# CVMI-Lab/HybridNeuralRendering

Measured on AMD Instinct MI355X. Metric: rays/sec (fwd render) scene0241_01 at 1/2/4/8 GPU; PSNR delta vs ref, higher is better.
Workload: dtype f32

## Files before the change

### hybridneuralrendering_amd/csrc/aggregate.hip

```cpp
#include "hnr_common.h"
#include "hnr_launch.h"

namespace hnr {

__device__ __forceinline__ int count_neighbours(const int32_t *__restrict__ p, int K)
{
    int n = 0;
    while (n < K && p[n] >= 0) ++n;
    return n;
}

__global__ __launch_bounds__(1024) void plan_block_sum_kernel(const int32_t *__restrict__ work, const int32_t *__restrict__ pidx,
                                                              const unsigned long long *__restrict__ counts, int K,
                                                              int32_t *__restrict__ block_sums)
{
    __shared__ int s_a[16], s_b[16];
    const int n_items = (int)counts[HNR_CNT_SAMPLES];
    const int i = blockIdx.x * 1024 + threadIdx.x;
    int nb = i < n_items ? count_neighbours(pidx + (size_t)work[i] * K, K) : 0;
    int v = nb > 0;
    for (int o = 32; o > 0; o >>= 1) { nb += __shfl_xor(nb, o); v += __shfl_xor(v, o); }
    if ((threadIdx.x & 63) == 0) { s_a[threadIdx.x >> 6] = v; s_b[threadIdx.x >> 6] = nb; }
    __syncthreads();
    if (threadIdx.x == 0) {
// ... 485 lines not shown
            wv *= vm[u];
            if (a.frame_w) wv *= a.frame_w[v0 + u];
            fsum += f[u] * wv;
            wsum += wv;
        }
    }
    float *o = a.X7 + (size_t)s * a.ld7;
    if (lane < 45) {
        o[lane] = a.CF[(size_t)s * a.ldcf + lane];
        const bool drop = a.ray_drop && a.ray_drop[a.vs_item[s] / a.SR];
        o[45 + lane] = drop ? 0.f : hnr_div(fsum, wsum + 1e-6f);
    }
    }
}

struct FinalArgs {
    const float *Y; int ldy;
    const float *CF; int ldcf;
    const float *w_fin, *b_fin;
    const float *sigma;
    const int32_t *vs_item;
    const unsigned long long *counts;
    float *decoded;
};

__global__ __launch_bounds__(256) void final_color_kernel(FinalArgs a)
{
    const int lane = threadIdx.x & 63, l16 = lane & 15, sub = lane >> 4;
    const int n_valid = (int)a.counts[HNR_CNT_SAMPLES_VALID];
    float w[3][8];
#pragma unroll
    for (int j = 0; j < 3; ++j)
#pragma unroll
        for (int e = 0; e < 8; ++e) w[j][e] = a.w_fin[j * 128 + 8 * l16 + e];
    const float b0 = a.b_fin[0], b1 = a.b_fin[1], b2 = a.b_fin[2];
    const bool yvec = a.ldy >= 48 && (a.ldy & 3) == 0 && (reinterpret_cast<uintptr_t>(a.Y) & 15) == 0;
    const int wave_g = (int)((blockIdx.x * (unsigned)blockDim.x + threadIdx.x) >> 6), n_waves = (int)((gridDim.x * (unsigned)blockDim.x) >> 6);
    for (int s0 = 4 * wave_g; s0 < n_valid; s0 += 4 * n_waves) {
        const int s = s0 + sub;
        const bool ok = s < n_valid;
        const size_t sc = ok ? (size_t)s : (size_t)(n_valid - 1);
        const float4 c0 = *reinterpret_cast<const float4 *>(a.CF + sc * a.ldcf + 8 * l16), c1 = *reinterpret_cast<const float4 *>(a.CF + sc * a.ldcf + 8 * l16 + 4);
        float x[8] = {c0.x, c0.y, c0.z, c0.w, c1.x, c1.y, c1.z, c1.w};
        if (yvec) {
            if (l16 < 6) {
                const float4 y0 = *reinterpret_cast<const float4 *>(a.Y + sc * a.ldy + 8 * l16), y1 = *reinterpret_cast<const float4 *>(a.Y + sc * a.ldy + 8 * l16 + 4);
                const float y[8] = {y0.x, y0.y, y0.z, y0.w, y1.x, y1.y, y1.z, y1.w};
#pragma unroll
                for (int e = 0; e < 8; ++e) if (8 * l16 + e < 45) x[e] = y[e] + x[e];
            }
        } else {
#pragma unroll
            for (int e = 0; e < 8; ++e) {
                const int c = 8 * l16 + e;
                if (c < 45) x[e] = a.Y[sc * a.ldy + c] + x[e];
            }
        }
        float r[3] = {0.f, 0.f, 0.f};
#pragma unroll
        for (int j = 0; j < 3; ++j) {
#pragma unroll
            for (int e = 0; e < 8; ++e) r[j] += x[e] * w[j][e];
            r[j] += __builtin_amdgcn_update_dpp(0.f, r[j], 0xB1, 0xf, 0xf, false);
            r[j] += __builtin_amdgcn_update_dpp(0.f, r[j], 0x4E, 0xf, 0xf, false);
            r[j] += __builtin_amdgcn_update_dpp(0.f, r[j], 0x141, 0xf, 0xf, false);
            r[j] += __builtin_amdgcn_update_dpp(0.f, r[j], 0x140, 0xf, 0xf, false);
        }
        if (l16 == 0 && ok) {
            float4 out;
            out.x = a.sigma[s];
            const float bb[3] = {b0, b1, b2};
            float rgb[3];
#pragma unroll
            for (int j = 0; j < 3; ++j) {
                const float sg = hnr_div(1.f, 1.f + expf(-(r[j] + bb[j])));
                rgb[j] = sg * (1.f + 2.f * 0.001f) - 0.001f;
            }
            out.y = rgb[0]; out.z = rgb[1]; out.w = rgb[2];
            reinterpret_cast<float4 *>(a.decoded)[a.vs_item[s]] = out;
        }
    }
}

struct CompositeArgs {
    const float *decoded;
    const float *loc_w;
    const int32_t *pidx;
    const int8_t *ray_mask;
    const int32_t *nsamp;
    const float *campos, *camrot, *bg;
    int R, SR, K;
    float vsize_z;
    int unit_mode;
    float *raycolor;
    float *opacity;
    float *is_bg;
    float *blend_w;
};

__global__ __launch_bounds__(256) void composite_kernel(CompositeArgs a)
{
    const int r = blockIdx.x * blockDim.x + threadIdx.x;
    if (r >= a.R) return;
    const float bg0 = a.bg[0], bg1 = a.bg[1], bg2 = a.bg[2];
    float *op = a.opacity + (size_t)r * a.SR;
    if (!a.ray_mask[r]) {
        a.raycolor[3 * (size_t)r] = bg0; a.raycolor[3 * (size_t)r + 1] = bg1; a.raycolor[3 * (size_t)r + 2] = bg2;
        a.is_bg[r] = 1.f;
        for (int s = 0; s < a.SR; ++s) { op[s] = 0.f; if (a.blend_w) a.blend_w[(size_t)r * a.SR + s] = 0.f; }
        return;
    }
    float cr[9];
#pragma unroll
    for (int i = 0; i < 9; ++i) cr[i] = a.camrot[i];
    const float cp[3] = {a.campos[0], a.campos[1], a.campos[2]};
    const int ns = a.nsamp ? a.nsamp[r] : a.SR;
    auto zc = [&](int s) {
        const float *p = a.loc_w + ((size_t)r * a.SR + s) * 3;
        const float q0 = s < ns ? p[0] : 0.f, q1 = s < ns ? p[1] : 0.f, q2 = s < ns ? p[2] : 0.f;
        const float s0 = __fsub_rn(q0, cp[0]), s1 = __fsub_rn(q1, cp[1]), s2 = __fsub_rn(q2, cp[2]);
        return __fadd_rn(__fadd_rn(__fmul_rn(cr[2], s0), __fmul_rn(cr[5], s1)), __fmul_rn(cr[8], s2));
    };
    float T = 1.f, c0 = 0.f, c1 = 0.f, c2 = 0.f;
    float zmax = zc(0);
    const int s_end = ns < a.SR ? ns : a.SR;
    for (int s = s_end; s < a.SR; ++s) { op[s] = 0.f; if (a.blend_w) a.blend_w[(size_t)r * a.SR + s] = 0.f; }
    for (int s = 0; s < s_end; ++s) {
        float dist;
        if (s + 1 < a.SR) {
            const float zn = fmaxf(zmax, zc(s + 1));
            dist = __fsub_rn(zn, zmax);
            zmax = zn;
        } else {
            dist = a.vsize_z;
        }
        if (dist < 1e-8f || (a.unit_mode && dist > 2.f * a.vsize_z)) dist = a.vsize_z;
        const bool valid = s < ns && a.pidx[((size_t)r * a.SR + s) * a.K] >= 0;
        const float4 d = reinterpret_cast<const float4 *>(a.decoded)[(size_t)r * a.SR + s];
        const float sigma = valid ? d.x : 0.f;
        const float rd = valid ? dist : 0.f;
        const float o = 1.f - expf(-sigma * rd);
        const float bw = o * T;
        c0 += d.y * bw; c1 += d.z * bw; c2 += d.w * bw;
        op[s] = o;
        if (a.blend_w) a.blend_w[(size_t)r * a.SR + s] = bw;
        T *= (1.f - o + 1e-10f);
    }
    a.raycolor[3 * (size_t)r] = c0 + bg0 * T;
    a.raycolor[3 * (size_t)r + 1] = c1 + bg1 * T;
    a.raycolor[3 * (size_t)r + 2] = c2 + bg2 * T;
    a.is_bg[r] = T;
}

__global__ __launch_bounds__(256) void ray_march_kernel(const float *__restrict__ ray_dist, const uint8_t *__restrict__ ray_valid,
                                                        const float *__restrict__ feat , const float *__restrict__ bg ,
                                                        int R, int SR, float *__restrict__ ray_color, float *__restrict__ opacity,
                                                        float *__restrict__ acc_t, float *__restrict__ blend_w, float *__restrict__ bg_t)
{
    const int r = blockIdx.x * blockDim.x + threadIdx.x;
    if (r >= R) return;
    float T = 1.f, c0 = 0.f, c1 = 0.f, c2 = 0.f;
    for (int s = 0; s < SR; ++s) {
        const size_t i = (size_t)r * SR + s;
        const float4 d = reinterpret_cast<const float4 *>(feat)[i];
        const float sigma = ray_valid[i] ? d.x : 0.f;
        const float o = 1.f - expf(-sigma * ray_dist[i]);
        const float w = o * T;
        opacity[i] = o; acc_t[i] = T; blend_w[i] = w;
        c0 += d.y * w; c1 += d.z * w; c2 += d.w * w;
        T *= (1.f - o + 1e-10f);
    }
    if (bg) { c0 += bg[0] * T; c1 += bg[1] * T; c2 += bg[2] * T; }
    ray_color[3 * (size_t)r] = c0; ray_color[3 * (size_t)r + 1] = c1; ray_color[3 * (size_t)r + 2] = c2;
    bg_t[r] = T;
}

struct ProbeArgs {
    const float *opacity, *loc_w;
    const int32_t *pidx;
    const float *weight, *conf_c;
    const float *xyz, *emb, *conf, *pdir, *color;
    int F, R, SR, K;
    float *o_opacity, *o_loc, *o_far, *o_color, *o_dir, *o_conf, *o_emb;
};

__global__ __launch_bounds__(256) void probe_kernel(ProbeArgs a)
{
    const int64_t t = (int64_t)blockIdx.x * blockDim.x + threadIdx.x;
    const int r = (int)(t >> 3), sub = (int)(t & 7);
    if (r >= a.R) return;
    int best = 0;
    float bo = a.opacity[(size_t)r * a.SR];
    for (int s = 1; s < a.SR; ++s) {
        const float o = a.opacity[(size_t)r * a.SR + s];
        if (o > bo) { bo = o; best = s; }
    }
    const size_t item = (size_t)r * a.SR + best;
    const float lx = a.loc_w[3 * item], ly = a.loc_w[3 * item + 1], lz = a.loc_w[3 * item + 2];
    float far = INFINITY, acc_c[3] = {0.f, 0.f, 0.f}, acc_d[3] = {0.f, 0.f, 0.f}, acc_f = 0.f;
    float acc_e[4] = {0.f, 0.f, 0.f, 0.f};
    for (int k = 0; k < a.K; ++k) {
        const int raw = a.pidx[item * a.K + k];
        const int pid = raw < 0 ? 0 : raw;
        const float w = a.weight[item * a.K + k] * a.conf_c[item * a.K + k];
        const float dx = a.xyz[3 * (size_t)pid] - lx, dy = a.xyz[3 * (size_t)pid + 1] - ly, dz = a.xyz[3 * (size_t)pid + 2] - lz;
        far = fminf(far, sqrtf(dx * dx + dy * dy + dz * dz));
#pragma unroll
        for (int j = 0; j < 3; ++j) {
            acc_c[j] += a.color[3 * (size_t)pid + j] * w;
            acc_d[j] += a.pdir[3 * (size_t)pid + j] * w;
        }
        acc_f += a.conf[pid] * w;
#pragma unroll
        for (int q = 0; q < 4; ++q) {
            const int c = sub + 8 * q;
            if (c < a.F) acc_e[q] += a.emb[(size_t)pid * a.F + c] * w;
        }
    }
#pragma unroll
    for (int q = 0; q < 4; ++q) {
        const int c = sub + 8 * q;
        if (c < a.F) a.o_emb[(size_t)r * a.F + c] = acc_e[q];
    }
    if (sub == 0) {
        a.o_opacity[r] = bo; a.o_far[r] = far; a.o_conf[r] = acc_f;
        a.o_loc[3 * (size_t)r] = lx; a.o_loc[3 * (size_t)r + 1] = ly; a.o_loc[3 * (size_t)r + 2] = lz;
#pragma unroll
        for (int j = 0; j < 3; ++j) { a.o_color[3 * (size_t)r + j] = acc_c[j]; a.o_dir[3 * (size_t)r + j] = acc_d[j]; }
    }
}

__global__ __launch_bounds__(256) void gather_points_kernel(const int32_t *__restrict__ pidx, int64_t n, const float *__restrict__ xyz,
                                                            const float *__restrict__ emb, const float *__restrict__ conf,
                                                            const float *__restrict__ pdir, const float *__restrict__ color, int F,
                                                            const float *__restrict__ campos, const float *__restrict__ camrot,
                                                            float *__restrict__ o_color, float *__restrict__ o_dir,
                                                            float *__restrict__ o_conf, float *__restrict__ o_emb,
                                                            float *__restrict__ o_pers, float *__restrict__ o_xyz, uint8_t *__restrict__ o_mask)
{
    const int64_t e = ((int64_t)blockIdx.x * blockDim.x + threadIdx.x) >> 3;
    const int sub = threadIdx.x & 7;
    if (e >= n) return;
    const int raw = pidx[e];
    const int pid = raw < 0 ? 0 : raw;
    for (int c = sub; c < F; c += 8) o_emb[e * F + c] = emb[(size_t)pid * F + c];
    if (sub < 3) {
        o_color[e * 3 + sub] = color[3 * (size_t)pid + sub];
        o_dir[e * 3 + sub] = pdir[3 * (size_t)pid + sub];
        o_xyz[e * 3 + sub] = xyz[3 * (size_t)pid + sub];
    }
    if (sub == 3) {
        const float p[3] = {xyz[3 * (size_t)pid], xyz[3 * (size_t)pid + 1], xyz[3 * (size_t)pid + 2]};
        float pp[3];
        w2pers(p, campos, camrot, pp);
        o_pers[e * 3] = pp[0]; o_pers[e * 3 + 1] = pp[1]; o_pers[e * 3 + 2] = pp[2];
    }
    if (sub == 4) { o_conf[e] = conf[pid]; o_mask[e] = raw >= 0 ? 1 : 0; }
}

}

using namespace hnr;

extern "C" int hnr_gather_points(const int32_t *d_sample_pidx, int64_t n_entries, const float *d_xyz, const float *d_emb,
                                 const float *d_conf, const float *d_dir, const float *d_color, int F, const float *d_campos,
                                 const float *d_camrot, float *d_o_color, float *d_o_dir, float *d_o_conf, float *d_o_emb,
                                 float *d_o_xyz_pers, float *d_o_xyz, uint8_t *d_o_mask, void *stream)
{
    if (n_entries < 0 || F <= 0) { set_error("hnr_gather_points: bad sizes"); return HNR_ERR_BADARG; }
    if (n_entries == 0) return HNR_OK;
    if (!d_sample_pidx || !d_xyz || !d_emb || !d_conf || !d_dir || !d_color || !d_campos || !d_camrot || !d_o_color || !d_o_dir ||
        !d_o_conf || !d_o_emb || !d_o_xyz_pers || !d_o_xyz || !d_o_mask) {
        set_error("hnr_gather_points: NULL argument"); return HNR_ERR_BADARG;
    }
    gather_points_kernel<<<cdiv(n_entries * 8, 256), 256, 0, (hipStream_t)stream>>>(d_sample_pidx, n_entries, d_xyz, d_emb, d_conf, d_dir,
                                                                                   d_color, F, d_campos, d_camrot, d_o_color, d_o_dir,
                                                                                   d_o_conf, d_o_emb, d_o_xyz_pers, d_o_xyz, d_o_mask);
    HNR_LAUNCH_CHECK();
    return HNR_OK;
}

extern "C" int hnr_sample_plan(const int32_t *d_work, const int32_t *d_sample_pidx, const int64_t *d_counts, int K,
                               int max_items, int32_t *d_vs_item, int32_t *d_vs_off, int32_t *d_vs_cnt,
                               int cap_samples, int cap_rows, int32_t *d_scratch, int32_t *d_overflow, void *stream)
{
    if (!d_work || !d_sample_pidx || !d_counts || !d_vs_item || !d_vs_off || !d_vs_cnt || !d_scratch || !d_overflow ||
        K <= 0 || max_items < 0) {
        set_error("hnr_sample_plan: bad argument"); return HNR_ERR_BADARG;
    }
    hipStream_t st = (hipStream_t)stream;
    HNR_HIP_CHECK(hipMemsetAsync(d_overflow, 0, 4, st));
    if (max_items == 0) return HNR_OK;
    const int nb = cdiv(max_items, 1024);
    const unsigned long long *cnt = reinterpret_cast<const unsigned long long *>(d_counts);
    plan_block_sum_kernel<<<nb, 1024, 0, st>>>(d_work, d_sample_pidx, cnt, K, d_scratch);
    plan_scan_kernel<<<nb, 1024, 0, st>>>(d_work, d_sample_pidx, cnt, K, d_scratch, d_vs_item, d_vs_off, d_vs_cnt,
                                          cap_samples, cap_rows, d_overflow);
    HNR_LAUNCH_CHECK();
    return HNR_OK;
}

extern "C" int hnr_gather_rows(const float *d_xyz, const float *d_emb, const float *d_conf, const float *d_dir,
                               const float *d_color, int F, const int32_t *d_sample_pidx, const float *d_sample_loc_w,
                               const float *d_raydir, const float *d_campos, const float *d_camrot,
                               const int32_t *d_vs_item, const int32_t *d_vs_off, const int32_t *d_vs_cnt,
                               const int64_t *d_counts, int SR, int K, int cap_samples,
// ... 146 lines not shown
    float *s2a = s1 + (size_t)V * 6 * H1 * W1, *s2 = s2a + (size_t)V * 12 * H2 * W2;
    float *s3a = s2 + (size_t)V * 12 * H2 * W2, *s3 = s3a + (size_t)V * 24 * H3 * W3;
    static const int old_conv = knob("HNR_CONV_OLD", 0);
    auto conv = [&](const float *in, int Cin, int Hin, int Win, int cl, int cstride, int li, int Cout, int stride, int Hout, int Wout, float *out) {
        const int64_t total = (int64_t)V * Cout * Hout * Wout, pixels = (int64_t)V * Hout * Wout;
#define HNR_CONV_TILE(CIN_, CT_, CL_) \
        if (!old_conv && Cin == CIN_ && Cout % CT_ == 0 && cl == CL_) { \
            conv3x3_lrelu_tile_kernel<CIN_, CT_, CL_><<<dim3((unsigned)cdiv(pixels, 256), Cout / CT_), 256, 0, st>>>(in, Hin, Win, cstride, d_conv_w[li], d_conv_b[li], \
                                                                                                                 Cout, stride, Hout, Wout, slope, out, V); \
            return; }
        HNR_CONV_TILE(3, 6, 1) HNR_CONV_TILE(6, 6, 0) HNR_CONV_TILE(12, 6, 0) HNR_CONV_TILE(24, 6, 0)
#undef HNR_CONV_TILE
        conv3x3_lrelu_kernel<<<cdiv(total, 256), 256, 0, st>>>(in, Cin, Hin, Win, cl, cstride, d_conv_w[li], d_conv_b[li], Cout, stride,
                                                                Hout, Wout, slope, out, V);
    };
    conv(d_img, 3, H, W, 1, 3, 0, 6, 2, H1, W1, s1a);
    conv(s1a, 6, H1, W1, 0, 0, 1, 6, 1, H1, W1, s1);
    conv(s1, 6, H1, W1, 0, 0, 2, 12, 2, H2, W2, s2a);
    conv(s2a, 12, H2, W2, 0, 0, 3, 12, 1, H2, W2, s2);
    conv(s2, 12, H2, W2, 0, 0, 4, 24, 2, H3, W3, s3a);
    conv(s3a, 24, H3, W3, 0, 0, 5, 24, 1, H3, W3, s3);
    featmap_kernel<<<dim3((unsigned)cdiv((int64_t)V * H * W, 256), 4), 256, 0, st>>>(d_img, s1, s2, s3, V, H, W, H1, W1, H2, W2, H3, W3, d_featmap);
    HNR_LAUNCH_CHECK();
    return HNR_OK;
}

extern "C" int64_t hnr_image_features_scratch_elems(int V, int H, int W)
{
    auto o = [](int n) { return (n + 2 - 3) / 2 + 1; };
    const int64_t H1 = o(H), W1 = o(W), H2 = o((int)H1), W2 = o((int)W1), H3 = o((int)H2), W3 = o((int)W2);
    return 2 * (int64_t)V * (6 * H1 * W1 + 12 * H2 * W2 + 24 * H3 * W3);
}

extern "C" int hnr_proj_rows(const float *d_sample_loc_w, const int32_t *d_vs_item, const int64_t *d_counts, const float *d_w2c,
                             const float *d_intrinsic, const float *d_campos, const float *d_campos_nearest, const float *d_featmap,
                             int V, int H, int W, const float *d_CF, int ldcf, int cap_samples, float *d_X6, int ld6,
                             float *d_vmask, int32_t *d_row_sample, void *stream)
{
    const bool split = d_row_sample != nullptr;
    if (!d_sample_loc_w || !d_vs_item || !d_counts || !d_w2c || !d_intrinsic || !d_campos || !d_campos_nearest || !d_featmap ||
        (!split && !d_CF) || !d_X6 || !d_vmask || V <= 0 || ld6 < (split ? 48 : 176) || (ld6 & 3) || (!split && (ldcf < 128 || (ldcf & 3)))) {
        set_error("hnr_proj_rows: bad argument"); return HNR_ERR_BADARG;
    }
    if (cap_samples <= 0) return HNR_OK;
    ProjArgs a;
    a.loc_w = d_sample_loc_w; a.vs_item = d_vs_item; a.counts = reinterpret_cast<const unsigned long long *>(d_counts);
    a.w2c = d_w2c; a.Kmat = d_intrinsic; a.campos = d_campos; a.campos_n = d_campos_nearest; a.fm = d_featmap; a.H = H; a.W = W;
    a.CF = d_CF; a.ldcf = ldcf; a.V = V; a.cap = cap_samples; a.X6 = d_X6; a.ld6 = ld6; a.vmask = d_vmask; a.row_sample = d_row_sample;
    { const int need = cdiv((int64_t)V * cap_samples * 16, 256); proj_rows_kernel<<<need < 8192 ? need : 8192, 256, 0, (hipStream_t)stream>>>(a); }
    HNR_LAUNCH_CHECK();
    return HNR_OK;
}

__global__ void div_probe_kernel(const float *n, const float *d, int count, float *q_hnr, float *q_ieee)
{
    const int i = blockIdx.x * blockDim.x + threadIdx.x;
    if (i < count) { q_hnr[i] = hnr::hnr_div(n[i], d[i]); q_ieee[i] = n[i] / d[i]; }
}
extern "C" int hnr_div_probe(const float *d_num, const float *d_den, int n, float *d_q_hnr, float *d_q_ieee, void *stream)
{
    if (n < 0 || (n > 0 && (!d_num || !d_den || !d_q_hnr || !d_q_ieee))) { set_error("hnr_div_probe: bad argument"); return HNR_ERR_BADARG; }
    if (n == 0) return HNR_OK;
    div_probe_kernel<<<cdiv(n, 256), 256, 0, (hipStream_t)stream>>>(d_num, d_den, n, d_q_hnr, d_q_ieee);
    HNR_LAUNCH_CHECK();
    return HNR_OK;
}

__global__ void div_probe2_kernel(const float *__restrict__ p, const float *__restrict__ c, float o, int count, int32_t *__restrict__ cell_hnr, int32_t *__restrict__ cell_ieee,
                                  double *__restrict__ q64_hnr, double *__restrict__ q64_ieee)
{
    const int i = blockIdx.x * blockDim.x + threadIdx.x;
    if (i >= count) return;
    cell_hnr[i] = hnr::cell_coord(p[i], o, c[i]);
    const float q = __fsub_rn(p[i], o) / c[i];
    cell_ieee[i] = (q > -2.0e9f && q < 2.0e9f) ? (int)floorf(q) : INT32_MIN;
    const double n = (double)p[i] * 1.0000001192092896, d = (double)c[i] * 3.0000000000000004;
    q64_hnr[i] = hnr::hnr_div64(n, d); q64_ieee[i] = n / d;
}
extern "C" int hnr_div_probe2(const float *d_p, const float *d_c, float origin, int n, int32_t *d_cell_hnr, int32_t *d_cell_ieee, double *d_q64_hnr, double *d_q64_ieee,
                              void *stream)
{
    if (n < 0 || (n > 0 && (!d_p || !d_c || !d_cell_hnr || !d_cell_ieee || !d_q64_hnr || !d_q64_ieee))) { set_error("hnr_div_probe2: bad argument"); return HNR_ERR_BADARG; }
    if (n == 0) return HNR_OK;
    div_probe2_kernel<<<cdiv(n, 256), 256, 0, (hipStream_t)stream>>>(d_p, d_c, origin, n, d_cell_hnr, d_cell_ieee, d_q64_hnr, d_q64_ieee);
    HNR_LAUNCH_CHECK();
    return HNR_OK;
}

extern "C" int hnr_proj_pixels(const float *d_sample_loc_w, const int32_t *d_vs_item, const int64_t *d_counts, const float *d_w2c,
                               const float *d_intrinsic, int V, int H, int W, int cap_samples, int32_t *d_pix, void *stream)
{
    if (!d_sample_loc_w || !d_vs_item || !d_counts || !d_w2c || !d_intrinsic || !d_pix || V <= 0 || H <= 0 || W <= 0) {
        set_error("hnr_proj_pixels: bad argument"); return HNR_ERR_BADARG;
    }
    if (cap_samples <= 0) return HNR_OK;
    const int need = cdiv((int64_t)V * cap_samples, 256);
    proj_pixels_kernel<<<need < 8192 ? need : 8192, 256, 0, (hipStream_t)stream>>>(d_sample_loc_w, d_vs_item, reinterpret_cast<const unsigned long long *>(d_counts), d_w2c,
                                                                                      d_intrinsic, V, H, W, cap_samples, d_pix);
    HNR_LAUNCH_CHECK();
    return HNR_OK;
}

extern "C" int hnr_merge(const float *d_X6, int ld6, const float *d_Hm, int ldh, const float *d_w_last, const float *d_b_last,
                         const float *d_vmask, const float *d_frame_w, const float *d_CF, int ldcf, const int64_t *d_counts,
                         int V, int cap_samples, float *d_X7, int ld7, const uint8_t *d_ray_drop, const int32_t *d_vs_item, int SR,
                         void *stream)
{
    if (!d_X6 || !d_Hm || !d_w_last || !d_b_last || !d_vmask || !d_CF || !d_counts || !d_X7 || ldh < 64 || ld7 < 90 ||
        (d_ray_drop && (!d_vs_item || SR <= 0))) {
        set_error("hnr_merge: bad argument"); return HNR_ERR_BADARG;
    }
    if (cap_samples <= 0) return HNR_OK;
    MergeArgs a;
    a.X6 = d_X6; a.ld6 = ld6; a.Hm = d_Hm; a.ldh = ldh; a.w_last = d_w_last; a.b_last = d_b_last; a.vmask = d_vmask;
    a.frame_w = d_frame_w; a.CF = d_CF; a.ldcf = ldcf; a.counts = reinterpret_cast<const unsigned long long *>(d_counts);
    a.V = V; a.cap = cap_samples; a.X7 = d_X7; a.ld7 = ld7; a.ray_drop = d_ray_drop; a.vs_item = d_vs_item; a.SR = SR;
    { const int need = cdiv((int64_t)cap_samples * 64, 256); merge_kernel<<<need < 8192 ? need : 8192, 256, 0, (hipStream_t)stream>>>(a); }
    HNR_LAUNCH_CHECK();
    return HNR_OK;
}

extern "C" int hnr_final_color(const float *d_Y, int ldy, const float *d_CF, int ldcf, const float *d_w_fin, const float *d_b_fin,
                               const float *d_sigma, const int32_t *d_vs_item, const int64_t *d_counts, int cap_samples,
                               float *d_decoded, void *stream)
{
    if (!d_Y || !d_CF || !d_w_fin || !d_b_fin || !d_sigma || !d_vs_item || !d_counts || !d_decoded || ldy < 45 || ldcf < 128 || (ldcf & 3) ||
        ((uintptr_t)d_CF & 15)) {
        set_error("hnr_final_color: bad argument (NULL pointer, ldy < 45, ldcf < 128 or not a multiple of 4, colour feature not 16-B aligned)"); return HNR_ERR_BADARG;
    }
    if (cap_samples <= 0) return HNR_OK;
    FinalArgs a;
    a.Y = d_Y; a.ldy = ldy; a.CF = d_CF; a.ldcf = ldcf; a.w_fin = d_w_fin; a.b_fin = d_b_fin; a.sigma = d_sigma;
    a.vs_item = d_vs_item; a.counts = reinterpret_cast<const unsigned long long *>(d_counts); a.decoded = d_decoded;
    { const int need = cdiv((int64_t)cap_samples * 16, 256); final_color_kernel<<<need < 8192 ? need : 8192, 256, 0, (hipStream_t)stream>>>(a); }
    HNR_LAUNCH_CHECK();
    return HNR_OK;
}

extern "C" int hnr_composite(const float *d_decoded, const float *d_sample_loc_w, const int32_t *d_sample_pidx,
                             const int8_t *d_ray_mask, const int32_t *d_ray_nsamp, const float *d_campos, const float *d_camrot, const float *d_bg_color,
                             int R, int SR, int K, float vsize_z, int raydist_mode_unit, float *d_raycolor, float *d_opacity,
                             float *d_is_background, float *d_blend_weight, void *stream)
{
    if (R < 0 || SR <= 0 || K <= 0) { set_error("hnr_composite: bad sizes"); return HNR_ERR_BADARG; }
    if (R == 0) return HNR_OK;
    if (!d_decoded || !d_sample_loc_w || !d_sample_pidx || !d_ray_mask || !d_campos || !d_camrot || !d_bg_color || !d_raycolor ||
        !d_opacity || !d_is_background) {
        set_error("hnr_composite: NULL argument"); return HNR_ERR_BADARG;
    }
    CompositeArgs a;
    a.decoded = d_decoded; a.loc_w = d_sample_loc_w; a.pidx = d_sample_pidx; a.ray_mask = d_ray_mask; a.nsamp = d_ray_nsamp; a.campos = d_campos;
    a.camrot = d_camrot; a.bg = d_bg_color; a.R = R; a.SR = SR; a.K = K; a.vsize_z = vsize_z; a.unit_mode = raydist_mode_unit;
    a.raycolor = d_raycolor; a.opacity = d_opacity; a.is_bg = d_is_background; a.blend_w = d_blend_weight;
    composite_kernel<<<cdiv(R, 256), 256, 0, (hipStream_t)stream>>>(a);
    HNR_LAUNCH_CHECK();
    return HNR_OK;
}

extern "C" int hnr_ray_march(const float *d_ray_dist, const uint8_t *d_ray_valid, const float *d_features, const float *d_bg_color, int R,
                             int SR, float *d_ray_color, float *d_opacity, float *d_acc_transmission, float *d_blend_weight,
                             float *d_bg_transmission, void *stream)
{
    if (R < 0 || SR <= 0) { set_error("hnr_ray_march: bad sizes"); return HNR_ERR_BADARG; }
    if (R == 0) return HNR_OK;
    if (!d_ray_dist || !d_ray_valid || !d_features || !d_ray_color || !d_opacity || !d_acc_transmission || !d_blend_weight || !d_bg_transmission) {
        set_error("hnr_ray_march: NULL argument"); return HNR_ERR_BADARG;
    }
    ray_march_kernel<<<cdiv(R, 256), 256, 0, (hipStream_t)stream>>>(d_ray_dist, d_ray_valid, d_features, d_bg_color, R, SR, d_ray_color, d_opacity,
                                                                    d_acc_transmission, d_blend_weight, d_bg_transmission);
    HNR_LAUNCH_CHECK();
    return HNR_OK;
}

extern "C" int hnr_probe_outputs(const float *d_opacity, const float *d_sample_loc_w, const int32_t *d_sample_pidx, const float *d_weight,
                                 const float *d_conf_coefficient, const float *d_xyz, const float *d_emb, const float *d_conf, const float *d_dir,
                                 const float *d_color, int F, int R, int SR, int K, float *d_max_opacity, float *d_max_loc_w, float *d_far_dist,
                                 float *d_avg_color, float *d_avg_dir, float *d_avg_conf, float *d_avg_emb, void *stream)
{
    if (R < 0 || SR <= 0 || K <= 0 || F <= 0 || F > 32) { set_error("hnr_probe_outputs: bad sizes (F <= 32)"); return HNR_ERR_BADARG; }
    if (R == 0) return HNR_OK;
    if (!d_opacity || !d_sample_loc_w || !d_sample_pidx || !d_weight || !d_conf_coefficient || !d_xyz || !d_emb || !d_conf || !d_dir || !d_color ||
        !d_max_opacity || !d_max_loc_w || !d_far_dist || !d_avg_color || !d_avg_dir || !d_avg_conf || !d_avg_emb) {
        set_error("hnr_probe_outputs: NULL argument"); return HNR_ERR_BADARG;
    }
    ProbeArgs a;
    a.opacity = d_opacity; a.loc_w = d_sample_loc_w; a.pidx = d_sample_pidx; a.weight = d_weight; a.conf_c = d_conf_coefficient; a.xyz = d_xyz;
    a.emb = d_emb; a.conf = d_conf; a.pdir = d_dir; a.color = d_color; a.F = F; a.R = R; a.SR = SR; a.K = K; a.o_opacity = d_max_opacity;
    a.o_loc = d_max_loc_w; a.o_far = d_far_dist; a.o_color = d_avg_color; a.o_dir = d_avg_dir; a.o_conf = d_avg_conf; a.o_emb = d_avg_emb;
    probe_kernel<<<cdiv((int64_t)R * 8, 256), 256, 0, (hipStream_t)stream>>>(a);
    HNR_LAUNCH_CHECK();
    return HNR_OK;
}

namespace hnr {
int point_rows_dc(const float *d_emb, const int32_t *d_ids, int n_cap, const long long *d_n, float *d_E, int lde, hipStream_t st)
{
    if (n_cap <= 0) return HNR_OK;
    const int64_t total = (int64_t)n_cap * (32 / 4 + 3 * 32);
    int blocks = cdiv(total, 256);
    if (blocks > 256 * 16) blocks = 256 * 16;
    point_rows_kernel<32><<<blocks, 256, 0, st>>>(d_emb, d_ids, n_cap, d_E, lde, d_n);
    HNR_LAUNCH_CHECK();
    return HNR_OK;
}
}
```

### hybridneuralrendering_amd/csrc/chain_ws.hip

```cpp
#include <utility>

#include "chain_defs.h"
#include "hnr_launch.h"

namespace hnr {

constexpr int CW_CST = ch_lds_exch(4) + 2048;
constexpr int CW_CST_FLOATS = CH_META_DESCALE + 4;
constexpr int CW_DSUM = CW_CST + ((CW_CST_FLOATS * 4 + 15) & ~15);
constexpr int CW_HMAX = CW_DSUM + 4 * 32 * 4 * 4;
constexpr int cw_lds_bytes() { return CW_HMAX + 5 * 512; }

#define CW_LOAD_FRAG(N_, rsrc_, voff_, soff_, IMM_) asm volatile("buffer_load_dwordx4 a[%2:%3], %0, %1, %4 offen offset:%5" :: "v"(voff_), "s"(rsrc_), "n"(N_), "n"((N_) + 3), "s"(soff_), "n"(IMM_))
template <int N> __device__ __forceinline__ void cw_mfma(f32x16 &acc, const u32x4 &x)
{
    asm volatile("v_mfma_f32_32x32x16_f16 %0, a[%2:%3], %1, %0" : "+v"(acc) : "v"(x), "n"(N), "n"(N + 3));
}
template <int N> __device__ __forceinline__ void cw_mfma_first(f32x16 &acc, const u32x4 &x)
{
    asm volatile("v_mfma_f32_32x32x16_f16 %0, a[%2:%3], %1, 0" : "=&v"(acc) : "v"(x), "n"(N), "n"(N + 3));
}
__device__ __forceinline__ void cw_mfma_vw(f32x16 &acc, const u32x4 &w, const u32x4 &x)
{
    asm volatile("v_mfma_f32_32x32x16_f16 %0, %1, %2, %0" : "+v"(acc) : "v"(w), "v"(x));
// ... 466 lines not shown
            if (ms == 0) {
                if (PR == 3) ex4 = CW_AT_F4(q_dsr, 0);
                const int ls = (j >> (3 - kc_e)) + (4 << kc_e) * PR;
                const bool st = (j & ((8 >> kc_e) - 1)) == 0;
                x5_voff = st ? (ls * a.ld5 + col0) * 4 : 0x40000000;
                x5_flag = kc_e > 0 ? 0.f : 1.f;
                x5_flag2 = kc_e > 1 ? 0.f : 1.f;
                if constexpr (TR) x5m = 0.f;
                if constexpr (TR) x5_take = (st && to.first + CW_KEEP(ls) < to.end) ? 1.f : 0.f;
            } else if (ms < 33) {
                const int d = (ms - 1) >> 2, t = (ms - 1) & 3, c = d >> 2, e0i = 4 * (d & 3), kb = d & 1;
                if (t == 0)
                    asm volatile("v_mul_f32 %0, %4, %8\n\tv_mul_f32 %1, %5, %8\n\tv_mul_f32 %2, %6, %8\n\tv_mul_f32 %3, %7, %8"
                                 : "=&v"(kf[kb][0]), "=&v"(kf[kb][1]), "=&v"(kf[kb][2]), "=&v"(kf[kb][3])
                                 : "v"(acc[se][c][e0i]), "v"(acc[se][c][e0i + 1]), "v"(acc[se][c][e0i + 2]), "v"(acc[se][c][e0i + 3]), "v"(wq_e));
                else if (t == 1)
                    asm volatile("v_add_f32_dpp %0, %0, %0 quad_perm:[1,0,3,2] row_mask:0xf bank_mask:0xf\n\tv_add_f32_dpp %1, %1, %1 quad_perm:[1,0,3,2] row_mask:0xf bank_mask:0xf\n\t"
                                 "v_add_f32_dpp %2, %2, %2 quad_perm:[1,0,3,2] row_mask:0xf bank_mask:0xf\n\tv_add_f32_dpp %3, %3, %3 quad_perm:[1,0,3,2] row_mask:0xf bank_mask:0xf"
                                 : "+v"(kf[kb][0]), "+v"(kf[kb][1]), "+v"(kf[kb][2]), "+v"(kf[kb][3]));
                else if (t == 2)
                    asm volatile("v_fmac_f32_dpp %0, %0, %4 quad_perm:[2,3,0,1] row_mask:0xf bank_mask:0xf\n\tv_fmac_f32_dpp %1, %1, %4 quad_perm:[2,3,0,1] row_mask:0xf bank_mask:0xf\n\t"
                                 "v_fmac_f32_dpp %2, %2, %4 quad_perm:[2,3,0,1] row_mask:0xf bank_mask:0xf\n\tv_fmac_f32_dpp %3, %3, %4 quad_perm:[2,3,0,1] row_mask:0xf bank_mask:0xf"
                                 : "+v"(kf[kb][0]), "+v"(kf[kb][1]), "+v"(kf[kb][2]), "+v"(kf[kb][3]) : "v"(x5_flag2));
                else {
                    asm volatile("v_fmac_f32_dpp %0, %0, %4 row_half_mirror row_mask:0xf bank_mask:0xf\n\tv_fmac_f32_dpp %1, %1, %4 row_half_mirror row_mask:0xf bank_mask:0xf\n\t"
                                 "v_fmac_f32_dpp %2, %2, %4 row_half_mirror row_mask:0xf bank_mask:0xf\n\tv_fmac_f32_dpp %3, %3, %4 row_half_mirror row_mask:0xf bank_mask:0xf"
                                 : "+v"(kf[kb][0]), "+v"(kf[kb][1]), "+v"(kf[kb][2]), "+v"(kf[kb][3]) : "v"(x5_flag));
                    __builtin_amdgcn_raw_buffer_store_b128(u32x4{__float_as_uint(kf[kb][0]), __float_as_uint(kf[kb][1]), __float_as_uint(kf[kb][2]), __float_as_uint(kf[kb][3])}, to.rs,
                                                           x5_voff + (32 * c + e0i) * 4, 0, 0);
                    if constexpr (TR) {
                        const float m4 = fmaxf(fmaxf(fabsf(kf[kb][0]), fabsf(kf[kb][1])), fmaxf(fabsf(kf[kb][2]), fabsf(kf[kb][3])));
                        x5m = fmaxf(x5m, __fmul_rn(m4, x5_take));
                    }
                }
            } else if (ms == 33) {
                if constexpr (TR) CW_HMAX_PUT(4, x5m);
                if (PR == 3) {
                    const float d = __fadd_rn(__fadd_rn(ex4.x, ex4.y), __fadd_rn(ex4.z, ex4.w));
                    __builtin_amdgcn_raw_buffer_store_b32(__float_as_uint(d), to.rs_aux, h == 0 ? (wave * 32 + j) * 4 : 0x40000000, 0, 0);
                }
            } else prefetch_next();
        }
    };

    auto b_read = [&](int rt, int s, int p) __attribute__((always_inline)) {
        const int off = s * SLOT + (rt * 2 + p) * 1024;
        return off < 65536 ? CW_AT(const u32x4, q_b0, off) : off < 131072 ? CW_AT(const u32x4, q_b1, off - 65536) : CW_AT(const u32x4, q_b2, off - 131072);
    };

    TileOut to_fin = tile_out(-1);
    CW_REFRESH(0);
    bq[0] = read_cst(3, 0); bq[1] = read_cst(3, 1); aq[0] = read_cst(4, 0); aq[1] = read_cst(4, 1);
    bf[0][0] = b_read(0, 0, 0); bf[0][1] = b_read(0, 0, 1);
    for (int tile = t_first; tile < t_end; tile += t_step) {
        ++n_my;
        const int tile_next = tile + t_step;
        const int tile_nx = tile_next < t_end ? tile_next : tile;
        const TileOut to_cur = tile_out(tile);
        CW_REFRESH(0);
        bf[1][0] = b_read(0, 1, 0); bf[1][1] = b_read(0, 1, 1);
        cw_static_for<16>([&](auto Pc) __attribute__((always_inline)) {
            constexpr int P = decltype(Pc)::value;
            constexpr int L = P >> 2, rt = P & 3, S = cw_steps(L), G0 = cw_goff(P);
            constexpr int PP = (P + 15) & 15, PL = PP >> 2, PR = PP & 3, sm = rt & 1;
            constexpr int T = 6 * S, H = T / 2;
            const TileOut &to_e = P == 0 ? to_fin : to_cur;
            if (DB >= 2) { const long long t_ = clock64(); tm[(P + 15) & 15] += t_ - t_prev; t_prev = t_; if (P == 2) tmf[3] += t_ - tf_prev; if (P == 1) tf_prev = t_; }
            if constexpr (P != 0) CW_REFRESH(P);
            if (P == 6) {
#pragma unroll
                for (int c = 0; c < 2; ++c)
#pragma unroll
                    for (int p = 0; p < 2; ++p)
                        wx[c][p] = __builtin_bit_cast(u32x4, __builtin_amdgcn_raw_buffer_load_b128(wsrd, woff + (c * 2 + p) * 1024, CH_W2 + 16 * CH_WSTEP, 0));
            }
            if (P == 13) load_ids(tile_nx, pid_n);
            if (P == 1) load_rest(tile);
            __builtin_amdgcn_sched_barrier(0);
            cw_static_for<6 * S>([&](auto kc) __attribute__((always_inline)) {
                constexpr int slot = decltype(kc)::value, it = slot / 6, s = cw_korder(L, it), g = (slot % 6) >> 1, c = slot & 1;
                if (slot == H) {
                    if constexpr (P == 15) { constexpr int d_ = cw_dma_count(0, 15, TR); if constexpr (d_ <= 63) cw_wait_vm<d_>(); }
                    if constexpr (P == 2) { constexpr int d_ = cw_dma_count(3, 2, TR); if constexpr (d_ <= 63) cw_wait_vm<d_>(); }
                    if (DB >= 2 && P == 1) { const long long t_ = clock64(); tmf[0] += t_ - tf_prev; tf_prev = t_; }
                    cw_lds_barrier();
                    if (DB >= 2 && P == 1) { const long long t_ = clock64(); tmf[1] += t_ - tf_prev; tf_prev = t_; }
                    if constexpr (L == 3) dma_image(tile_nx, rt);
                    if constexpr (!TR && L == 0 && rt < 3) load_table(pid[rt + 1], tv[TR ? 0 : (rt + 1) & 1]);
                    if constexpr (TR && L == 0 && rt >= 1) load_table(pid[rt], tv[0]);
                    if constexpr (P == 14) load_table(pid_n[0], tv[0]);
                    if (DB >= 2 && P == 1) { const long long t_ = clock64(); tmf[2] += t_ - tf_prev; tf_prev = t_; }
                    __builtin_amdgcn_sched_barrier(0);
                }
                constexpr int wp = g == 0 ? 1 : 0, xp_ = g == 1 ? 1 : 0;
                constexpr int ring = (G0 + it) % 3;
                if constexpr (rt == 0 && g == 0 && c == 0 && s < 16) {
                    constexpr int n_ = cw_need_count(32 * L + s, P, slot, TR) + (P == 0 ? 8 : 0);
                    if constexpr (n_ <= (TR ? 63 : 56)) cw_wait_vm<n_>();
                }
                constexpr int A0 = 16 * (s < 16 ? s : 0) + 4 * wp + 8 * c;
                if constexpr (DB == 4) { if (slot < 2) { acc[sm][c] = f32x16{} + bf[ring][xp_][0]; } }
                else if constexpr (L == 2 && s == 16) cw_mfma_vw(acc[sm][c], wx[c][wp], bf[ring][xp_]);
                else if constexpr (slot < 2) cw_mfma_first<A0>(acc[sm][c], bf[ring][xp_]);
                else cw_mfma<A0>(acc[sm][c], bf[ring][xp_]);
                __builtin_amdgcn_sched_barrier(0);
                if constexpr (g < 2 && c == 0 && G0 + it + 2 < CW_GTOT) {
                    constexpr int i2 = it + 2 >= S ? it + 2 - S : it + 2, P2 = it + 2 >= S ? P + 1 : P;
                    if constexpr (P2 < 16 && i2 < cw_steps((P2 & 15) >> 2)) bf[(G0 + it + 2) % 3][g] = b_read(P2 & 3, cw_korder((P2 & 15) >> 2, i2), g);
                }
                if constexpr (g < 2 && c == 0 && P == 15 && it == 15) bf[0][g] = b_read(0, 0, g);
                { constexpr int blk = cw_issue(P, slot); if constexpr (blk >= 0) CW_LOAD_W(blk >> 5, blk & 31); }
                if (DB != 3) epilogue_piece(PL, PR, S, slot, to_e);
                __builtin_amdgcn_sched_barrier(0);
            });
        });
        wq_fin = wq[3]; to_fin = to_cur;
#pragma unroll
        for (int rt = 0; rt < 4; ++rt) pid[rt] = pid_n[rt];
    }
    CW_REFRESH(0);
    cw_static_for<6 * CH_S0>([&](auto kc) __attribute__((always_inline)) {
        constexpr int slot = decltype(kc)::value;
        if (slot == (6 * CH_S0) / 2) cw_lds_barrier();
        epilogue_piece(3, 3, CH_S0, slot, to_fin);
    });
    asm volatile("s_waitcnt vmcnt(0)" ::: "memory");
    if constexpr (TR) {
        __syncthreads();
        float *exch = reinterpret_cast<float *>(lds + ch_lds_exch(4));
#pragma unroll
        for (int l = 0; l < 5; ++l) {
            float m = tid < 128 ? CW_LDS(float, CW_HMAX + l * 512 + 4 * tid) : 0.f;
            for (int o = 32; o > 0; o >>= 1) m = fmaxf(m, __shfl_xor(m, o));
            if (lane == 0) exch[4 * l + wave] = m;
        }
        __syncthreads();
        if (tid < 5) {
            const float m = fmaxf(fmaxf(exch[4 * tid], exch[4 * tid + 1]), fmaxf(exch[4 * tid + 2], exch[4 * tid + 3]));
            unsigned *dst = tid < 4 ? (a.hmax ? a.hmax + tid : nullptr) : a.x5max;
            if (dst && m > 0.f) atomicMax(dst, __float_as_uint(m));
        }
    }
    if (DB >= 2 && blockIdx.x == 0 && lane == 0 && a.dbg) {
        long long *o = reinterpret_cast<long long *>(a.dbg) + 4 * 1024 + wave * 16;
        for (int i = 0; i < 16; ++i) o[i] = tm[i];
        if (wave == 0) { long long *o2 = reinterpret_cast<long long *>(a.dbg) + 4 * 1024 + 64; for (int i = 0; i < 4; ++i) o2[i] = tmf[i]; }
    }
    if (DB >= 2 && tid == 0 && a.dbg) {
        long long *o = reinterpret_cast<long long *>(a.dbg) + 4 * (size_t)blockIdx.x;
        o[0] = clock64() - t_start; o[1] = wall_clock64() - w_start; o[2] = n_my; o[3] = 0;
    }
}

__global__ __launch_bounds__(128) void chain_sigma_kernel(ChainArgs a)
{
    const ChainClasses cls = chain_classes(a.counts, a.cap_samples);
    const int tile = blockIdx.x;
    if (tile >= cls.n_tiles) return;
    const int lane = threadIdx.x & 63, rt = threadIdx.x >> 5, j = lane & 31;
    const char *aux = a.aux + ((size_t)tile * 4 + rt) * CH_AUX_GROUP;
    const float d = a.dsig[(size_t)tile * 128 + threadIdx.x], wq = reinterpret_cast<const float *>(aux + 128)[j];
    const float alpha_b = reinterpret_cast<const float *>(a.wimg + CH_META)[4 * 256 + 256];
    const int kc = chain_tile_class(cls, tile);
    float sg = __fmul_rn(chain_softplus_m1(__fadd_rn(d, alpha_b)), wq);
    sg = __fadd_rn(sg, __builtin_amdgcn_update_dpp(0.f, sg, 0xB1, 0xf, 0xf, false));
    { const float g = __builtin_amdgcn_update_dpp(0.f, sg, 0x4E, 0xf, 0xf, false); sg = __fadd_rn(sg, kc > 1 ? 0.f : g); }
    { const float g = __builtin_amdgcn_update_dpp(0.f, sg, 0x141, 0xf, 0xf, false); sg = __fadd_rn(sg, kc > 0 ? 0.f : g); }
    const int s_sig = chain_tile_first(cls, tile, kc) + (4 << kc) * rt + (j >> (3 - kc));
    if ((j & ((8 >> kc) - 1)) == 0 && s_sig < chain_class_end(cls, kc)) a.sigma[s_sig] = sg;
}

int launch_chain_ws(const ChainArgs &a, int grid, hipStream_t st, int mode)
{
    int rc;
#define HNR_CHAIN_WS_MODE(M_) launch_lds<chain_ws_kernel<M_>>(grid, 256, cw_lds_bytes(), st, a)
    switch (mode) {
    default: rc = HNR_CHAIN_WS_MODE(0); break;
    case 1: rc = HNR_CHAIN_WS_MODE(1); break;
    case 2: rc = HNR_CHAIN_WS_MODE(2); break;
    case 8: rc = HNR_CHAIN_WS_MODE(8); break;
#ifdef HNR_CHAIN_WS_PROBES
    case 3: rc = HNR_CHAIN_WS_MODE(3); break;
    case 4: rc = HNR_CHAIN_WS_MODE(4); break;
    case 5: rc = HNR_CHAIN_WS_MODE(5); break;
    case 6: rc = HNR_CHAIN_WS_MODE(6); break;
    case 7: rc = HNR_CHAIN_WS_MODE(7); break;
#endif
    }
#undef HNR_CHAIN_WS_MODE
    if (rc != HNR_OK) return rc;
    const int tiles = (a.cap_samples + 15) / 16 + 2;
    chain_sigma_kernel<<<tiles, 128, 0, st>>>(a);
    HNR_LAUNCH_CHECK();
    return HNR_OK;
}

}
```

Measured before the change: 8.342 million.

## Split composite across lane groups per ray and loop sigma kernel over tiles

Adds a composite kernel that assigns G lanes (8 by default) to each ray. The lanes load samples in parallel and exchange distances and opacities through shuffles to run the sequential transmittance scan, which replaces the one-thread-per-ray serial loop. Separately, the sigma epilogue becomes a grid-stride kernel capped at 16 blocks per CU, with four tiles' loads issued before compute to cut launch size and hide latency. Both are on by default and the old paths stay reachable via knobs. The serial shuffle loops add per-sample overhead, and the max-z distance chain is computed redundantly in every lane.

```diff
diff --git a/hybridneuralrendering_amd/csrc/aggregate.hip b/hybridneuralrendering_amd/csrc/aggregate.hip
--- a/hybridneuralrendering_amd/csrc/aggregate.hip
+++ b/hybridneuralrendering_amd/csrc/aggregate.hip
@@ -661,6 +661,82 @@
     a.is_bg[r] = T;
 }
 
+template <int G>
+__global__ __launch_bounds__(256) void composite_group_kernel(CompositeArgs a)
+{
+    const int64_t t = (int64_t)blockIdx.x * blockDim.x + threadIdx.x;
+    const int r = (int)(t / G), sub = (int)(t & (G - 1));
+    if (r >= a.R) return;
+    const float bg0 = a.bg[0], bg1 = a.bg[1], bg2 = a.bg[2];
+    float *op = a.opacity + (size_t)r * a.SR;
+    float *bwp = a.blend_w ? a.blend_w + (size_t)r * a.SR : nullptr;
+    if (!a.ray_mask[r]) {
+        if (sub == 0) {
+            a.raycolor[3 * (size_t)r] = bg0; a.raycolor[3 * (size_t)r + 1] = bg1; a.raycolor[3 * (size_t)r + 2] = bg2;
+            a.is_bg[r] = 1.f;
+        }
+        for (int s = sub; s < a.SR; s += G) { op[s] = 0.f; if (bwp) bwp[s] = 0.f; }
+        return;
+    }
+    const float cr2 = a.camrot[2], cr5 = a.camrot[5], cr8 = a.camrot[8];
+    const float cp[3] = {a.campos[0], a.campos[1], a.campos[2]};
+    const int ns = a.nsamp ? a.nsamp[r] : a.SR;
+    auto zc = [&](int s) {
+        const float *p = a.loc_w + ((size_t)r * a.SR + s) * 3;
+        const float q0 = s < ns ? p[0] : 0.f, q1 = s < ns ? p[1] : 0.f, q2 = s < ns ? p[2] : 0.f;
+        const float s0 = __fsub_rn(q0, cp[0]), s1 = __fsub_rn(q1, cp[1]), s2 = __fsub_rn(q2, cp[2]);
+        return __fadd_rn(__fadd_rn(__fmul_rn(cr2, s0), __fmul_rn(cr5, s1)), __fmul_rn(cr8, s2));
+    };
+    const int s_end = ns < a.SR ? ns : a.SR;
+    for (int s = s_end + sub; s < a.SR; s += G) { op[s] = 0.f; if (bwp) bwp[s] = 0.f; }
+    float T = 1.f, c0 = 0.f, c1 = 0.f, c2 = 0.f;
+    float zmax = zc(0);
+    for (int base = 0; base < s_end; base += G) {
+        const int s = base + sub, n = s_end - base < G ? s_end - base : G;
+        const bool mine = s < s_end;
+        float4 d = make_float4(0.f, 0.f, 0.f, 0.f);
+        bool valid = false;
+        float z1 = 0.f;
+        if (mine) {
+            valid = a.pidx[((size_t)r * a.SR + s) * a.K] >= 0;
+            d = reinterpret_cast<const float4 *>(a.decoded)[(size_t)r * a.SR + s];
+            if (s + 1 < a.SR) z1 = zc(s + 1);
+        }
+        float dist_me = 0.f;
+        for (int j = 0; j < n; ++j) {
+            const float z_next = __shfl(z1, j, G);
+            float dist;
+            if (base + j + 1 < a.SR) {
+                const float zn = fmaxf(zmax, z_next);
+                dist = __fsub_rn(zn, zmax);
+                zmax = zn;
+            } else {
+                dist = a.vsize_z;
+            }
+            if (dist < 1e-8f || (a.unit_mode && dist > 2.f * a.vsize_z)) dist = a.vsize_z;
+            if (j == sub) dist_me = dist;
+        }
+        const float sigma = valid ? d.x : 0.f;
+        const float rd = valid ? dist_me : 0.f;
+        const float o = 1.f - expf(-sigma * rd);
+        float bw_me = 0.f;
+        for (int j = 0; j < n; ++j) {
+            const float oj = __shfl(o, j, G), y = __shfl(d.y, j, G), z = __shfl(d.z, j, G), w = __shfl(d.w, j, G);
+            const float bw = oj * T;
+            c0 += y * bw; c1 += z * bw; c2 += w * bw;
+            if (j == sub) bw_me = bw;
+            T *= (1.f - oj + 1e-10f);
+        }
+        if (mine) { op[s] = o; if (bwp) bwp[s] = bw_me; }
+    }
+    if (sub == 0) {
+        a.raycolor[3 * (size_t)r] = c0 + bg0 * T;
+        a.raycolor[3 * (size_t)r + 1] = c1 + bg1 * T;
+        a.raycolor[3 * (size_t)r + 2] = c2 + bg2 * T;
+        a.is_bg[r] = T;
+    }
+}
+
 __global__ __launch_bounds__(256) void ray_march_kernel(const float *__restrict__ ray_dist, const uint8_t *__restrict__ ray_valid,
                                                         const float *__restrict__ feat , const float *__restrict__ bg ,
                                                         int R, int SR, float *__restrict__ ray_color, float *__restrict__ opacity,
@@ -1113,7 +1189,10 @@
     a.decoded = d_decoded; a.loc_w = d_sample_loc_w; a.pidx = d_sample_pidx; a.ray_mask = d_ray_mask; a.nsamp = d_ray_nsamp; a.campos = d_campos;
     a.camrot = d_camrot; a.bg = d_bg_color; a.R = R; a.SR = SR; a.K = K; a.vsize_z = vsize_z; a.unit_mode = raydist_mode_unit;
     a.raycolor = d_raycolor; a.opacity = d_opacity; a.is_bg = d_is_background; a.blend_w = d_blend_weight;
-    composite_kernel<<<cdiv(R, 256), 256, 0, (hipStream_t)stream>>>(a);
+    const int lanes = knob_now("HNR_COMPOSITE_LANES", 8);
+    if (lanes == 8) composite_group_kernel<8><<<cdiv((int64_t)R * 8, 256), 256, 0, (hipStream_t)stream>>>(a);
+    else if (lanes == 16) composite_group_kernel<16><<<cdiv((int64_t)R * 16, 256), 256, 0, (hipStream_t)stream>>>(a);
+    else composite_kernel<<<cdiv(R, 256), 256, 0, (hipStream_t)stream>>>(a);
     HNR_LAUNCH_CHECK();
     return HNR_OK;
 }
diff --git a/hybridneuralrendering_amd/csrc/chain_ws.hip b/hybridneuralrendering_amd/csrc/chain_ws.hip
--- a/hybridneuralrendering_amd/csrc/chain_ws.hip
+++ b/hybridneuralrendering_amd/csrc/chain_ws.hip
@@ -642,15 +642,9 @@
     }
 }
 
-__global__ __launch_bounds__(128) void chain_sigma_kernel(ChainArgs a)
-{
-    const ChainClasses cls = chain_classes(a.counts, a.cap_samples);
-    const int tile = blockIdx.x;
-    if (tile >= cls.n_tiles) return;
+__device__ __forceinline__ void chain_sigma_tile(const ChainArgs &a, const ChainClasses &cls, int tile, float d, float wq, float alpha_b)
+{
     const int lane = threadIdx.x & 63, rt = threadIdx.x >> 5, j = lane & 31;
-    const char *aux = a.aux + ((size_t)tile * 4 + rt) * CH_AUX_GROUP;
-    const float d = a.dsig[(size_t)tile * 128 + threadIdx.x], wq = reinterpret_cast<const float *>(aux + 128)[j];
-    const float alpha_b = reinterpret_cast<const float *>(a.wimg + CH_META)[4 * 256 + 256];
     const int kc = chain_tile_class(cls, tile);
     float sg = __fmul_rn(chain_softplus_m1(__fadd_rn(d, alpha_b)), wq);
     sg = __fadd_rn(sg, __builtin_amdgcn_update_dpp(0.f, sg, 0xB1, 0xf, 0xf, false));
@@ -658,6 +652,42 @@
     { const float g = __builtin_amdgcn_update_dpp(0.f, sg, 0x141, 0xf, 0xf, false); sg = __fadd_rn(sg, kc > 0 ? 0.f : g); }
     const int s_sig = chain_tile_first(cls, tile, kc) + (4 << kc) * rt + (j >> (3 - kc));
     if ((j & ((8 >> kc) - 1)) == 0 && s_sig < chain_class_end(cls, kc)) a.sigma[s_sig] = sg;
+}
+__device__ __forceinline__ float chain_sigma_wq(const ChainArgs &a, int tile)
+{
+    const char *aux = a.aux + ((size_t)tile * 4 + (threadIdx.x >> 5)) * CH_AUX_GROUP;
+    return reinterpret_cast<const float *>(aux + 128)[threadIdx.x & 31];
+}
+
+__global__ __launch_bounds__(128) void chain_sigma_kernel(ChainArgs a)
+{
+    const ChainClasses cls = chain_classes(a.counts, a.cap_samples);
+    const int tile = blockIdx.x;
+    if (tile >= cls.n_tiles) return;
+    const float d = a.dsig[(size_t)tile * 128 + threadIdx.x], wq = chain_sigma_wq(a, tile);
+    const float alpha_b = reinterpret_cast<const float *>(a.wimg + CH_META)[4 * 256 + 256];
+    chain_sigma_tile(a, cls, tile, d, wq, alpha_b);
+}
+
+__global__ __launch_bounds__(128) void chain_sigma_loop_kernel(ChainArgs a)
+{
+    const ChainClasses cls = chain_classes(a.counts, a.cap_samples);
+    const float alpha_b = reinterpret_cast<const float *>(a.wimg + CH_META)[4 * 256 + 256];
+    const int step = (int)gridDim.x;
+    for (int t0 = blockIdx.x; t0 < cls.n_tiles; t0 += 4 * step) {
+        float d[4], wq[4];
+#pragma unroll
+        for (int u = 0; u < 4; ++u) {
+            const int tile = t0 + u * step;
+            d[u] = 0.f; wq[u] = 0.f;
+            if (tile < cls.n_tiles) { d[u] = a.dsig[(size_t)tile * 128 + threadIdx.x]; wq[u] = chain_sigma_wq(a, tile); }
+        }
+#pragma unroll
+        for (int u = 0; u < 4; ++u) {
+            const int tile = t0 + u * step;
+            if (tile < cls.n_tiles) chain_sigma_tile(a, cls, tile, d[u], wq[u], alpha_b);
+        }
+    }
 }
 
 int launch_chain_ws(const ChainArgs &a, int grid, hipStream_t st, int mode)
@@ -680,7 +710,9 @@
 #undef HNR_CHAIN_WS_MODE
     if (rc != HNR_OK) return rc;
     const int tiles = (a.cap_samples + 15) / 16 + 2;
-    chain_sigma_kernel<<<tiles, 128, 0, st>>>(a);
+    const int loop_blocks = 16 * device_num_cus();
+    if (knob_now("HNR_SIGMA_LOOP", 1) != 0) chain_sigma_loop_kernel<<<tiles < loop_blocks ? tiles : loop_blocks, 128, 0, st>>>(a);
+    else chain_sigma_kernel<<<tiles, 128, 0, st>>>(a);
     HNR_LAUNCH_CHECK();
     return HNR_OK;
 }
```

New measurement: 8.424 million, median of 6. About the same (+1.0%).
